# rusty-fast-solvers/rusty-compression

Hardware: AMD Instinct MI355X
Metric: GB/s + compressions/sec, 8192x8192 f64 rank-128 rSVD+ID (higher is better)
Workload: dtype f64

## Files before the change

### bindings/rust/src/ffi.rs

```rust
#![allow(non_camel_case_types)]
use std::os::raw::{c_char, c_void};

pub type rc_status = i32;
pub const RC_OK: rc_status = 0;
pub const RC_LINALG_ERROR: rc_status = 1;
pub const RC_COMPRESSION_ERROR: rc_status = 2;
pub const RC_LAYOUT_ERROR: rc_status = 3;
pub const RC_PIVOTED_QR_ERROR: rc_status = 4;
pub const RC_INVALID_ARGUMENT: rc_status = 5;
pub const RC_RUNTIME_ERROR: rc_status = 6;

pub const RC_PERM_COL: i32 = 0;
pub const RC_PERM_ROW: i32 = 1;
pub const RC_PERM_COLINV: i32 = 2;
pub const RC_PERM_ROWINV: i32 = 3;
pub const RC_VPERM_INV: i32 = 0;
pub const RC_VPERM_NOINV: i32 = 1;

pub const RC_OPT_TALL_SKINNY_FAST_PATH: i32 = 1;
pub const RC_OPT_WIDE_LAZY_QRCP: i32 = 2;
pub const RC_OPT_WIDE_COOP_QRCP: i32 = 3;
pub const RC_OPT_POWER_ITERATION_FIXED: i32 = 4;
pub const RC_OPT_FORK_BRANCHES: i32 = 5;
pub const RC_OPT_BLOCKED_QRCP: i32 = 6;
pub const RC_OPT_CONCURRENCY_HINT: i32 = 7;
pub const RC_OPT_COOP_PANEL: i32 = 8;
pub const RC_OPT_KERNEL_SLOTS: i32 = 9;
pub const RC_OPT_FUSED_CONSUMERS: i32 = 10;

#[repr(C)]
#[derive(Clone, Copy)]
pub struct rc_matrix {
    pub data: *mut c_void,
    pub rows: i64,
    pub cols: i64,
    pub row_stride: i64,
    pub col_stride: i64,
}

#[repr(C)]
#[derive(Clone, Copy)]
pub struct rc_rsvd_id_out {
    pub range_q: rc_matrix,
    pub u: rc_matrix,
    pub s: *mut c_void,
    pub vt: rc_matrix,
    pub qr_q: rc_matrix,
    pub qr_r: rc_matrix,
    pub qr_ind: *mut i64,
    pub id_c: rc_matrix,
    pub id_z: rc_matrix,
}

#[repr(C)]
#[derive(Clone, Copy)]
pub struct rc_complex32 {
    pub re: f32,
    pub im: f32,
}
#[repr(C)]
#[derive(Clone, Copy)]
pub struct rc_complex64 {
    pub re: f64,
    pub im: f64,
}

#[repr(C)]
pub struct rc_context {
    _private: [u8; 0],
}
#[repr(C)]
pub struct rc_comm {
    _private: [u8; 0],
}
pub type rc_host_all_gather_fn = Option<unsafe extern "C" fn(user: *mut c_void, send: *const c_void, recv: *mut c_void, bytes_per_rank: usize) -> i32>;
pub type rc_host_all_reduce_sum_fn = Option<unsafe extern "C" fn(user: *mut c_void, buf: *mut c_void, count: usize, elem_size: i32) -> i32>;
pub type rc_operator_product_fn = Option<unsafe extern "C" fn(user: *mut c_void, ctx: *mut rc_context, x: rc_matrix, y: rc_matrix) -> i32>;
#[repr(C)]
#[derive(Clone, Copy)]
pub struct rc_operator {
    pub rows: i64,
// ... 220 lines not shown
```

### include/rusty_compression_amd.h

```cpp
#ifndef RUSTY_COMPRESSION_AMD_H
#define RUSTY_COMPRESSION_AMD_H

#include <stddef.h>
#include <stdint.h>

#ifdef __cplusplus
extern "C" {
#endif

#define RC_ABI_VERSION 1

typedef int32_t rc_status;
enum {
    RC_OK = 0,
    RC_LINALG_ERROR = 1,
    RC_COMPRESSION_ERROR = 2,
    RC_LAYOUT_ERROR = 3,
    RC_PIVOTED_QR_ERROR = 4,
    RC_INVALID_ARGUMENT = 5,
    RC_RUNTIME_ERROR = 6
};

typedef struct rc_matrix {
    void *data;
    int64_t rows;
    int64_t cols;
    int64_t row_stride;
    int64_t col_stride;
} rc_matrix;

typedef struct rc_context rc_context;

enum { RC_COMPRESS_ADAPTIVE = 0, RC_COMPRESS_RANK = 1 };
enum { RC_PERM_COL = 0, RC_PERM_ROW = 1, RC_PERM_COLINV = 2, RC_PERM_ROWINV = 3 };
enum { RC_VPERM_INV = 0, RC_VPERM_NOINV = 1 };

int32_t rc_abi_version(void);
rc_status rc_create(rc_context **ctx, int32_t device, void *hip_stream);
rc_status rc_destroy(rc_context *ctx);
rc_status rc_set_stream(rc_context *ctx, void *hip_stream);
rc_status rc_stream_create(int32_t device, void **hip_stream);
rc_status rc_stream_destroy(int32_t device, void *hip_stream);
rc_status rc_synchronize(rc_context *ctx);
rc_status rc_synchronize_all(rc_context *const *ctxs, int32_t n);
rc_status rc_reserve_workspace(rc_context *ctx, size_t bytes);
const char *rc_last_error_message(const rc_context *ctx);

rc_status rc_device_malloc(rc_context *ctx, size_t bytes, void **ptr);
rc_status rc_device_free(rc_context *ctx, void *ptr);
rc_status rc_memcpy_h2d(rc_context *ctx, void *dst_dev, const void *src_host, size_t bytes);
rc_status rc_memcpy_d2h(rc_context *ctx, void *dst_host, const void *src_dev, size_t bytes);

rc_status rc_graph_begin_capture(rc_context *ctx);
rc_status rc_graph_end_capture(rc_context *ctx, void **graph_exec);
rc_status rc_graph_launch(rc_context *ctx, void *graph_exec);
rc_status rc_graph_destroy(rc_context *ctx, void *graph_exec);

enum { RC_OPT_TALL_SKINNY_FAST_PATH = 1, RC_OPT_WIDE_LAZY_QRCP = 2, RC_OPT_WIDE_COOP_QRCP = 3, RC_OPT_POWER_ITERATION_FIXED = 4, RC_OPT_FORK_BRANCHES = 5,
       RC_OPT_BLOCKED_QRCP = 6, RC_OPT_CONCURRENCY_HINT = 7, RC_OPT_COOP_PANEL = 8, RC_OPT_KERNEL_SLOTS = 9, RC_OPT_FUSED_CONSUMERS = 10 };
rc_status rc_set_option(rc_context *ctx, int32_t option, int64_t value);
rc_status rc_get_health(rc_context *ctx, int32_t *word);

rc_status rc_profile_enable(rc_context *ctx, int32_t on);
rc_status rc_profile_reset(rc_context *ctx);
rc_status rc_profile_count(rc_context *ctx, int32_t *n);
rc_status rc_profile_get(rc_context *ctx, int32_t i, char *name, int32_t name_cap, double *total_ms, int64_t *calls);

const char *rc_last_gemm_kernel_name(const rc_context *ctx);

rc_status rc_random_gaussian_f64(rc_context *ctx, rc_matrix out, uint64_t seed, uint64_t offset);
rc_status rc_random_gaussian_f32(rc_context *ctx, rc_matrix out, uint64_t seed, uint64_t offset);
rc_status rc_random_bits_u32(rc_context *ctx, uint32_t *out, int64_t n, uint64_t seed, uint64_t word_offset);

rc_status rc_matmat_f64(rc_context *ctx, rc_matrix a, rc_matrix x, rc_matrix y);
rc_status rc_matmat_f32(rc_context *ctx, rc_matrix a, rc_matrix x, rc_matrix y);
rc_status rc_conj_matmat_f64(rc_context *ctx, rc_matrix a, rc_matrix x, rc_matrix y);
rc_status rc_conj_matmat_f32(rc_context *ctx, rc_matrix a, rc_matrix x, rc_matrix y);
rc_status rc_gemm_f64(rc_context *ctx, int32_t trans_a, int32_t trans_b, double alpha, rc_matrix a, rc_matrix b, double beta, rc_matrix c);
rc_status rc_gemm_f32(rc_context *ctx, int32_t trans_a, int32_t trans_b, float alpha, rc_matrix a, rc_matrix b, float beta, rc_matrix c);
rc_status rc_rel_diff_fro_f64(rc_context *ctx, rc_matrix first, rc_matrix second, double *out);
rc_status rc_rel_diff_fro_f32(rc_context *ctx, rc_matrix first, rc_matrix second, float *out);

rc_status rc_invert_permutation(rc_context *ctx, const int64_t *perm, int64_t n, int64_t *inverse);
rc_status rc_apply_permutation_matrix_f64(rc_context *ctx, int32_t mode, rc_matrix in, const int64_t *perm, int64_t perm_len, rc_matrix out);
rc_status rc_apply_permutation_matrix_f32(rc_context *ctx, int32_t mode, rc_matrix in, const int64_t *perm, int64_t perm_len, rc_matrix out);
rc_status rc_apply_permutation_vector_f64(rc_context *ctx, int32_t mode, rc_matrix in, const int64_t *perm, int64_t perm_len, rc_matrix out);
rc_status rc_apply_permutation_vector_f32(rc_context *ctx, int32_t mode, rc_matrix in, const int64_t *perm, int64_t perm_len, rc_matrix out);

rc_status rc_pivoted_qr_f64(rc_context *ctx, rc_matrix a, rc_matrix q, rc_matrix r, int64_t *ind);
rc_status rc_pivoted_qr_f32(rc_context *ctx, rc_matrix a, rc_matrix q, rc_matrix r, int64_t *ind);
rc_status rc_pivoted_lq_f64(rc_context *ctx, rc_matrix a, rc_matrix l, rc_matrix q, int64_t *ind);
rc_status rc_pivoted_lq_f32(rc_context *ctx, rc_matrix a, rc_matrix l, rc_matrix q, int64_t *ind);

rc_status rc_geqp3_f64(rc_context *ctx, rc_matrix a, int64_t kmax, int64_t *jpvt, double *tau);
rc_status rc_geqp3_f32(rc_context *ctx, rc_matrix a, int64_t kmax, int64_t *jpvt, float *tau);
rc_status rc_orgqr_f64(rc_context *ctx, rc_matrix a, const double *tau, int64_t k, rc_matrix q);
rc_status rc_orgqr_f32(rc_context *ctx, rc_matrix a, const float *tau, int64_t k, rc_matrix q);
rc_status rc_trsm_upper_f64(rc_context *ctx, rc_matrix t, rc_matrix b);
rc_status rc_trsm_upper_f32(rc_context *ctx, rc_matrix t, rc_matrix b);

rc_status rc_compute_svd_f64(rc_context *ctx, rc_matrix a, rc_matrix u, double *s, rc_matrix vt);
rc_status rc_compute_svd_f32(rc_context *ctx, rc_matrix a, rc_matrix u, float *s, rc_matrix vt);

rc_status rc_rank_by_tolerance_f64(rc_context *ctx, rc_matrix tri, double tol, int64_t *rank);
rc_status rc_rank_by_tolerance_f32(rc_context *ctx, rc_matrix tri, double tol, int64_t *rank);
rc_status rc_qr_to_mat_f64(rc_context *ctx, rc_matrix q, rc_matrix r, const int64_t *ind, rc_matrix out);
rc_status rc_qr_to_mat_f32(rc_context *ctx, rc_matrix q, rc_matrix r, const int64_t *ind, rc_matrix out);
rc_status rc_lq_to_mat_f64(rc_context *ctx, rc_matrix l, rc_matrix q, const int64_t *ind, rc_matrix out);
rc_status rc_lq_to_mat_f32(rc_context *ctx, rc_matrix l, rc_matrix q, const int64_t *ind, rc_matrix out);
rc_status rc_qr_column_id_f64(rc_context *ctx, rc_matrix q, rc_matrix r, const int64_t *ind, rc_matrix c, rc_matrix z);
rc_status rc_qr_column_id_f32(rc_context *ctx, rc_matrix q, rc_matrix r, const int64_t *ind, rc_matrix c, rc_matrix z);
rc_status rc_lq_row_id_f64(rc_context *ctx, rc_matrix l, rc_matrix q, const int64_t *ind, rc_matrix x, rc_matrix r_rows);
// ... 192 lines not shown
```

### rusty_compression_amd/_lib.py

```python
from __future__ import annotations

import ctypes
import os
import re
import threading
from typing import Dict, Optional, Tuple

_HERE = os.path.dirname(os.path.abspath(__file__))
LIB_PATH = os.path.join(_HERE, "librusty_compression_amd.so")
HEADER_PATH = os.path.join(os.path.dirname(_HERE), "include", "rusty_compression_amd.h")

RC_OPT_TALL_SKINNY_FAST_PATH = 1
RC_OPT_WIDE_LAZY_QRCP = 2
RC_OPT_WIDE_COOP_QRCP = 3
RC_OPT_POWER_ITERATION_FIXED = 4
RC_OPT_FORK_BRANCHES = 5
RC_OPT_BLOCKED_QRCP = 6
RC_OPT_CONCURRENCY_HINT = 7
RC_OPT_COOP_PANEL = 8
RC_OPT_KERNEL_SLOTS = 9
RC_OPT_FUSED_CONSUMERS = 10
RC_OK, RC_LINALG_ERROR, RC_COMPRESSION_ERROR, RC_LAYOUT_ERROR, RC_PIVOTED_QR_ERROR, RC_INVALID_ARGUMENT, RC_RUNTIME_ERROR = range(7)


class RustyCompressionError(Exception):
    """Base of the error enum of the reference (src/types.rs:11-21)."""


class LinalgError(RustyCompressionError):
    pass


class CompressionError(RustyCompressionError):
    """`Could not compress to desired tolerance` (src/types.rs:15-16)."""


class LayoutError(RustyCompressionError):
    pass


class PivotedQRError(RustyCompressionError):
    pass


class HipRuntimeError(RustyCompressionError):
    pass


_STATUS_EXC = {
    RC_LINALG_ERROR: LinalgError,
    RC_COMPRESSION_ERROR: CompressionError,
    RC_LAYOUT_ERROR: LayoutError,
    RC_PIVOTED_QR_ERROR: PivotedQRError,
    RC_INVALID_ARGUMENT: AssertionError,
    RC_RUNTIME_ERROR: HipRuntimeError,
}


class rc_matrix(ctypes.Structure):
    _fields_ = [
        ("data", ctypes.c_void_p),
        ("rows", ctypes.c_int64),
        ("cols", ctypes.c_int64),
        ("row_stride", ctypes.c_int64),
        ("col_stride", ctypes.c_int64),
    ]


class rc_rsvd_id_out(ctypes.Structure):
    _fields_ = [
        ("range_q", rc_matrix),
        ("u", rc_matrix),
        ("s", ctypes.c_void_p),
        ("vt", rc_matrix),
# ... 162 lines not shown
```

### rusty_compression_amd/csrc/kernels_qr.hip

```cpp
#include "rc_common.hpp"
#include "rc_device.hpp"

namespace rc {

static __host__ __device__ inline int64_t cdiv(int64_t a, int64_t b) { return (a + b - 1) / b; }

template <typename T> struct Num;
template <> struct Num<double> {
    static __host__ __device__ inline double tol3z() { return 1.0536712127723509e-08; }
};
template <> struct Num<float> {
    static __host__ __device__ inline float tol3z() { return 2.44140625e-04f; }
};

template <typename T>
__device__ inline T wsum(T v) {
#pragma unroll
    for (int off = 32; off > 0; off >>= 1) v += __shfl_xor(v, off, 64);
    return v;
}

template <typename T, int TPC>
__device__ inline T group_sum(T v, T *sh ) {
    v = wsum(v);
    if (TPC == 256) {
        __syncthreads();
        if ((threadIdx.x & 63) == 0) sh[threadIdx.x >> 6] = v;
        __syncthreads();
        v = sh[0] + sh[1] + sh[2] + sh[3];
    }
    return v;
}

template <typename T>
__global__ __launch_bounds__(256) void k_qr_init(Mat<T> w, int pivot, int64_t *jpvt, T *vn1, T *vn2) {
    __shared__ T sh[4];
    for (int64_t j = blockIdx.x; j < w.cols; j += gridDim.x) {
        if (pivot) {
            const T *col = w.p + j * w.cs;
            T acc = 0;
            for (int64_t i = threadIdx.x; i < w.rows; i += 256) { T v = col[i]; acc += v * v; }
            acc = group_sum<T, 256>(acc, sh);
            if (threadIdx.x == 0) { T nrm = sqrt(acc); vn1[j] = nrm; vn2[j] = nrm; }
        }
        if (threadIdx.x == 0) jpvt[j] = j;
    }
}

template <typename T>
__global__ __launch_bounds__(1024) void k_qr_pivot_reflect(Mat<T> w, int64_t j, int pivot, int64_t *jpvt, T *vn1, T *vn2, T *tau) {
    __shared__ T shv[16];
    __shared__ long long shi[16];
    __shared__ T shs[16];
    const int tid = threadIdx.x, lane = tid & 63, wv = tid >> 6;
// ... 517 lines not shown
__global__ __launch_bounds__(256) void k_id_z(Mat<T> w, const int64_t *jpvt, int64_t k, Mat<T> z) {
    constexpr int NB = 16;
    __shared__ T tile[NB][NB + 1];
    const int64_t n = w.cols;
    const int64_t p = blockIdx.x * (int64_t)blockDim.x + threadIdx.x;
    const bool inside = p < n;
    const int64_t dc = inside ? jpvt[p] : 0;
    const bool active = inside && p >= k;
    const T *bcol = FROM_R ? w.p + (inside ? p : 0) * w.cs : w.p + dc * w.cs;
    const int64_t brs = FROM_R ? w.rs : 1;
    const int64_t nblk = (k + NB - 1) / NB;
    const int ti = threadIdx.x / NB, tj = threadIdx.x % NB;
    if (inside && p < k)
        for (int64_t i = 0; i < k; ++i) z.at(i, dc) = (i == p) ? (T)1 : (T)0;
    for (int64_t bi = nblk - 1; bi >= 0; --bi) {
        const int64_t r0 = bi * NB;
        T acc[NB];
#pragma unroll
        for (int ii = 0; ii < NB; ++ii) acc[ii] = (active && r0 + ii < k) ? bcol[(r0 + ii) * brs] : (T)0;
        for (int64_t bj = nblk - 1; bj >= bi; --bj) {
            const int64_t c0 = bj * NB;
            __syncthreads();
            {
                const int64_t i = r0 + ti, l = c0 + tj;
                tile[ti][tj] = (i < k && l < k && i <= l) ? (FROM_R ? w.at(i, l) : w.p[jpvt[l] * w.cs + i]) : (T)0;
            }
            __syncthreads();
            if (bj > bi) {
                T x[NB];
#pragma unroll
                for (int jj = 0; jj < NB; ++jj) x[jj] = (active && c0 + jj < k) ? z.at(c0 + jj, dc) : (T)0;
#pragma unroll
                for (int jj = 0; jj < NB; ++jj)
#pragma unroll
                    for (int ii = 0; ii < NB; ++ii) acc[ii] -= tile[ii][jj] * x[jj];
            } else {
#pragma unroll
                for (int ii = NB - 1; ii >= 0; --ii) {
                    if (r0 + ii < k) {
                        acc[ii] /= tile[ii][ii];
#pragma unroll
                        for (int i2 = 0; i2 < ii; ++i2) acc[i2] -= tile[i2][ii] * acc[ii];
                    }
                }
            }
        }
        if (active) {
#pragma unroll
            for (int ii = 0; ii < NB; ++ii)
                if (r0 + ii < k) z.at(r0 + ii, dc) = acc[ii];
        }
    }
}
template <typename T>
void column_id_from_qrcp(rc_context *c, Mat<T> a, Mat<T> w, int64_t k, const int64_t *jpvt, Mat<T> cm, Mat<T> z) {
    RC_REQUIRE(w.rs == 1 && a.rows == w.rows && a.cols == w.cols && cm.rows == a.rows && cm.cols == k && z.rows == k && z.cols == a.cols && k <= std::min(a.rows, a.cols),
               RC_INVALID_ARGUMENT, "column_id_from_qrcp: shape mismatch");
    if (a.cols == 0 || k == 0) return;
    ProfScope ps(c, "op:column_id_from_qrcp %lldx%lld k=%lld", (long long)a.rows, (long long)a.cols, (long long)k);
    hipLaunchKernelGGL((k_id_z<T, false>), dim3((unsigned)cdiv(a.cols, 256)), dim3(256), 0, c->stream, w, jpvt, k, z);
    gather_cols(c, a, jpvt, cm);
}
template <typename T>
void id_z_from_r(rc_context *c, Mat<T> r, int64_t k, const int64_t *ind, Mat<T> z) {
    RC_REQUIRE(r.rows == k && z.rows == k && z.cols == r.cols && k <= r.cols, RC_INVALID_ARGUMENT, "id_z_from_r: shape mismatch");
    if (r.cols == 0 || k == 0) return;
    ProfScope ps(c, "op:id_z_from_r k=%lld n=%lld", (long long)k, (long long)r.cols);
    hipLaunchKernelGGL((k_id_z<T, true>), dim3((unsigned)cdiv(r.cols, 256)), dim3(256), 0, c->stream, r, ind, k, z);
}

#define RC_INST(T)                                                                                         \
    template void column_id_from_qrcp<T>(rc_context *, Mat<T>, Mat<T>, int64_t, const int64_t *, Mat<T>, Mat<T>); \
    template void id_z_from_r<T>(rc_context *, Mat<T>, int64_t, const int64_t *, Mat<T>);                 \
    template void geqp3_inplace<T>(rc_context *, Mat<T>, int64_t, bool, int64_t *, T *, T *);             \
    template void extract_r<T>(rc_context *, Mat<T>, const int64_t *, Mat<T>);                             \
    template void form_q<T>(rc_context *, Mat<T>, const int64_t *, const T *, int64_t, Mat<T>);           \
    template void trsm_upper<T>(rc_context *, Mat<T>, Mat<T>);
RC_INST(double)
RC_INST(float)
#undef RC_INST

}

namespace rc {

template <typename T>
__global__ __launch_bounds__(256) void k_wq_init(Mat<T> qacc, Mat<T> rphys) {
    const int64_t tq = qacc.rows * qacc.cols, tr = rphys.rows * rphys.cols;
    for (int64_t e = blockIdx.x * (int64_t)blockDim.x + threadIdx.x; e < tq + tr; e += (int64_t)gridDim.x * blockDim.x) {
        if (e < tq) { int64_t i = e % qacc.rows, c2 = e / qacc.rows; qacc.p[c2 * qacc.cs + i] = (i == c2) ? (T)1 : (T)0; }
        else rphys.p[e - tq] = 0;
    }
}

template <typename T>
__global__ __launch_bounds__(1024) void k_wq_pivot(Mat<T> b, Mat<T> qacc, Mat<T> rphys, int64_t j, int64_t *jpvt, T *vn1, T *vn2, T *tau) {
    extern __shared__ __attribute__((aligned(16))) char smem_raw[];
    const int m = (int)b.rows;
    const int ldq = m | 1;
    long long *shi = reinterpret_cast<long long *>(smem_raw);
    T *shv = reinterpret_cast<T *>(shi + 16);
    T *Q = shv + 16;
    T *bvec = Q + (size_t)m * ldq;
    T *xvec = bvec + m;
    T *vvec = xvec + m;
    T *wvec = vvec + m;
    const int tid = threadIdx.x, lane = tid & 63, wv = tid >> 6;
    const int l8 = tid & 7, g8 = tid >> 3;
    const int64_t n = b.cols;
    const int jj = (int)j;
    for (int e = tid; e < (m - jj) * m; e += 1024) {
        const int i = jj + e / m, r = e % m;
        Q[i * ldq + r] = qacc.p[(int64_t)i * qacc.cs + r];
    }
    {
        T best = (T)-1;
        long long bi = 0x7fffffffffffffffLL;
        for (int64_t p = j + tid; p < n; p += 1024) {
            T v = fabs(vn1[p]);
            if (v > best) { best = v; bi = p; }
        }
// ... 225 lines not shown
```

### rusty_compression_amd/csrc/kernels_tsqr.hip

```cpp
#include "rc_common.hpp"
#include "rc_device.hpp"

namespace rc {

static __host__ __device__ inline int64_t cdiv(int64_t a, int64_t b) { return (a + b - 1) / b; }

template <typename T> struct TNum;
template <> struct TNum<double> {
    static __device__ inline double tol3z() { return 1.0536712127723509e-08; }
    static __device__ inline double tiny() { return 1e-300; }
};
template <> struct TNum<float> {
    static __device__ inline float tol3z() { return 2.44140625e-04f; }
    static __device__ inline float tiny() { return 1e-30f; }
};

template <typename T>
__device__ inline T wave_sum64(T v) {
#pragma unroll
    for (int off = 32; off > 0; off >>= 1) v += __shfl_xor(v, off, 64);
    return v;
}
template <typename T>
__device__ inline T row_sum16(T v) {
// ... 386 lines not shown

template <typename T>
void qrcp_small(rc_context *c, Mat<T> rin, int64_t kmax, bool pivot, int64_t *jpvt, Mat<T> rout, Mat<T> q2) {
    const int64_t n = rin.rows;
    RC_REQUIRE(rin.rows == rin.cols, RC_INVALID_ARGUMENT, "qrcp_small: square input required");
    const size_t lds = ((size_t)n * (n | 1) + 3 * (size_t)n) * sizeof(T) + (size_t)n * sizeof(int) + 64;
    RC_REQUIRE(lds <= 160 * 1024 - 1024 && n <= 208, RC_INVALID_ARGUMENT, "qrcp_small: n = %lld does not fit LDS", (long long)n);
    ProfScope ps(c, "op:qrcp_small n=%lld k=%lld", (long long)n, (long long)kmax);
#define RC_QS(NE, NT_)                                                                                                 \
    do {                                                                                                               \
        auto kern = k_qrcp_small<T, NE, NT_>;                                                                          \
        static bool attr_set[64] = {};                                                                                 \
        if (!attr_set[c->device & 63]) {                                                                               \
            RC_HIP(hipFuncSetAttribute(reinterpret_cast<const void *>(kern), hipFuncAttributeMaxDynamicSharedMemorySize, 160 * 1024 - 1024)); \
            attr_set[c->device & 63] = true;                                                                           \
        }                                                                                                              \
        hipLaunchKernelGGL(kern, dim3(1), dim3(NT_), lds, c->stream, rin, (int)kmax, pivot ? 1 : 0, jpvt, rout, q2);   \
    } while (0)
    static const int wide = [] { const char *e = getenv("RC_QRCP_SMALL_1024"); return e ? atoi(e) : 1; }();
    if (n <= 64) RC_QS(8, 512);
    else if (n <= 144 && wide) RC_QS(18, 1024);
    else if (n <= 144) RC_QS(18, 512);
    else RC_QS(26, 512);
#undef RC_QS
}

template <typename T>
__global__ __launch_bounds__(1024) void k_householder_signs(Mat<T> q, T *d) {
    extern __shared__ __attribute__((aligned(16))) char smem_raw[];
    const int k = (int)q.cols;
    const int ld = k | 1;
    T *W = reinterpret_cast<T *>(smem_raw);
    const int tid = threadIdx.x;
    for (int e = tid; e < k * k; e += 1024) {
        int i = e % k, cc = e / k;
        W[i * ld + cc] = q.at(i, cc);
    }
    __syncthreads();
    const int ti = tid >> 5, tc = tid & 31;
    for (int j = 0; j < k; ++j) {
        const T s = W[j * ld + j];
        const T dj = (s > (T)0) ? (T)-1 : (T)1;
        const T u = (T)1 + fabs(s);
        if (tid == 0) d[j] = dj;
        const T inv = -dj / u;
        for (int i = j + 1 + ti; i < k; i += 32) {
            const T li = W[i * ld + j] * inv;
            for (int cc = j + 1 + tc; cc < k; cc += 32) W[i * ld + cc] -= li * W[j * ld + cc];
        }
        __syncthreads();
    }
}
template <typename T>
__global__ __launch_bounds__(256) void k_scale_cols_rows(Mat<T> q, Mat<T> r, const T *d) {
    const int64_t tq = q.rows * q.cols, tr = r.rows * r.cols;
    for (int64_t e = blockIdx.x * (int64_t)blockDim.x + threadIdx.x; e < tq + tr; e += (int64_t)gridDim.x * blockDim.x) {
        if (e < tq) {
            int64_t j = e / q.rows, i = e - j * q.rows;
            if (d[j] < (T)0) q.at(i, j) = -q.at(i, j);
        } else {
            int64_t f = e - tq;
            int64_t i = f / r.cols, p = f - i * r.cols;
            if (d[i] < (T)0) r.at(i, p) = -r.at(i, p);
        }
    }
}

template <typename T>
static void householder_signs(rc_context *c, Mat<T> top, T *d) {
    const int64_t k = top.cols;
    const size_t lds = (size_t)k * (k | 1) * sizeof(T);
    RC_REQUIRE(top.rows >= k && lds <= 160 * 1024 - 1024, RC_INVALID_ARGUMENT, "sign fix: k = %lld does not fit LDS", (long long)k);
    auto kern = k_householder_signs<T>;
    static bool attr_set[64] = {};
    if (!attr_set[c->device & 63]) {
        RC_HIP(hipFuncSetAttribute(reinterpret_cast<const void *>(kern), hipFuncAttributeMaxDynamicSharedMemorySize, 160 * 1024 - 1024));
        attr_set[c->device & 63] = true;
    }
    hipLaunchKernelGGL(kern, dim3(1), dim3(1024), lds, c->stream, top, d);
}
template <typename T>
static void scale_cols_rows(rc_context *c, Mat<T> q, Mat<T> r, const T *d) {
    const int64_t total = q.rows * q.cols + r.rows * r.cols;
    hipLaunchKernelGGL(k_scale_cols_rows<T>, dim3((unsigned)std::min<int64_t>(cdiv(total, 256), 4096)), dim3(256), 0, c->stream, q, r, d);
}

template <typename T>
void householder_sign_fix(rc_context *c, Mat<T> q, Mat<T> r) {
    const int64_t k = q.cols;
    if (k == 0) return;
    RC_REQUIRE(q.rows >= k, RC_INVALID_ARGUMENT, "sign fix: q must be tall");
    ProfScope ps(c, "op:householder_sign_fix k=%lld", (long long)k);
    ArenaMark mark(c);
    T *d = c->alloc<T>((size_t)k);
    householder_signs<T>(c, q, d);
    scale_cols_rows<T>(c, q, r, d);
}

template <typename T>
void qrcp_tall_fast(rc_context *c, Mat<T> y, int64_t k, bool pivot, Mat<T> q, Mat<T> r, int64_t *ind, int *flag) {
    const int64_t m = y.rows, n = y.cols;
    ProfScope ps(c, "op:qrcp_tall_fast %lldx%lld k=%lld pivot=%d", (long long)m, (long long)n, (long long)k, pivot ? 1 : 0);
    ArenaMark mark(c);
    static const int fold = [] { const char *e = getenv("RC_TSQR_FOLD"); return e ? atoi(e) : 1; }();
    Mat<T> q1 = rowmajor(c->alloc<T>((size_t)m * even_ld(n)), m, n, even_ld(n));
    Mat<T> r1 = colmajor(c->alloc<T>((size_t)n * even_ld(n)), n, n, even_ld(n));
    Mat<T> r2i = rowmajor(c->alloc<T>((size_t)n * even_ld(n)), n, n, even_ld(n));
    if (fold) tsqr_cholqr2_factored<T>(c, y, q1, r2i, r1, flag);
    else tsqr_cholqr2<T>(c, y, q1, r1, flag);
    Mat<T> q2 = colmajor(c->alloc<T>((size_t)even_ld(n) * k), n, k, even_ld(n));
    Mat<T> rr = r.empty() ? rowmajor(c->alloc<T>((size_t)k * even_ld(n)), k, n, even_ld(n)) : r;
    qrcp_small<T>(c, r1, k, pivot, ind, rr, q2);
    Mat<T> qq = q.empty() ? rowmajor(c->alloc<T>((size_t)m * even_ld(k)), m, k, even_ld(k)) : q;
    if (!fold) {
        gemm<T>(c, 1, q1, q2, 0, qq);
        householder_sign_fix<T>(c, qq, rr);
        return;
    }
    Mat<T> w = colmajor(c->alloc<T>((size_t)even_ld(n) * k), n, k, even_ld(n));
    Mat<T> top = colmajor(c->alloc<T>((size_t)even_ld(k) * k), k, k, even_ld(k));
    T *d = c->alloc<T>((size_t)k);
    gemm<T>(c, 1, r2i, q2, 0, w);
    gemm<T>(c, 1, q1.sub(0, k, 0, n), w, 0, top);
    householder_signs<T>(c, top, d);
    scale_cols_rows<T>(c, w, rr, d);
    gemm<T>(c, 1, q1, w, 0, qq);
}

#define RC_INST(T)                                                                                               \
    template bool tsqr_supported<T>(int64_t, int64_t);                                                           \
    template void tsqr_cholqr2<T>(rc_context *, Mat<T>, Mat<T>, Mat<T>, int *);                                  \
    template void tsqr_cholqr2_factored<T>(rc_context *, Mat<T>, Mat<T>, Mat<T>, Mat<T>, int *);                 \
// ... 9 lines not shown
```

### rusty_compression_amd/csrc/rc_api.hip

```cpp
#include "rc_common.hpp"

#include <unistd.h>

#include <atomic>
#include <chrono>

#include <algorithm>
#include <cmath>

using namespace rc;

static constexpr size_t kAlign = 256;

void rc_context::retire_arena() {
    if (arena) {
        if (live_graphs > 0) retired.push_back(arena);
        else (void)hipFree(arena);
    }
    arena = nullptr;
    arena_size = 0;
}

void rc_context::swap_arena() {
    std::swap(arena, aux_arena.base);
// ... 1283 lines not shown
    if (e != hipSuccess) { ctx->last_error = hipGetErrorString(e); return RC_RUNTIME_ERROR; }
    ctx->capturing = true;
    return RC_OK;
}
rc_status rc_graph_end_capture(rc_context *ctx, void **graph_exec) {
    if (!ctx || !graph_exec) return RC_INVALID_ARGUMENT;
    DeviceGuard dg(ctx->device);
    *graph_exec = nullptr;
    hipGraph_t graph = nullptr;
    hipError_t e = hipStreamEndCapture(ctx->stream, &graph);
    ctx->capturing = false;
    if (e != hipSuccess || !graph) { ctx->last_error = std::string("hipStreamEndCapture: ") + hipGetErrorString(e); return RC_RUNTIME_ERROR; }
    hipGraphExec_t exec = nullptr;
    e = hipGraphInstantiate(&exec, graph, nullptr, nullptr, 0);
    (void)hipGraphDestroy(graph);
    if (e != hipSuccess) { ctx->last_error = std::string("hipGraphInstantiate: ") + hipGetErrorString(e); return RC_RUNTIME_ERROR; }
    *graph_exec = exec;
    ctx->live_graphs += 1;
    return RC_OK;
}
rc_status rc_graph_launch(rc_context *ctx, void *graph_exec) {
    if (!ctx || !graph_exec) return RC_INVALID_ARGUMENT;
    DeviceGuard dg(ctx->device);
    hipError_t e = hipGraphLaunch(static_cast<hipGraphExec_t>(graph_exec), ctx->stream);
    if (e != hipSuccess) { ctx->last_error = hipGetErrorString(e); return RC_RUNTIME_ERROR; }
    return RC_OK;
}
rc_status rc_graph_destroy(rc_context *ctx, void *graph_exec) {
    if (!ctx) return RC_INVALID_ARGUMENT;
    if (!graph_exec) return RC_OK;
    DeviceGuard dg(ctx->device);
    (void)hipStreamSynchronize(ctx->stream);
    (void)hipGraphExecDestroy(static_cast<hipGraphExec_t>(graph_exec));
    if (ctx->live_graphs > 0 && --ctx->live_graphs == 0) {
        for (void *p : ctx->retired) (void)hipFree(p);
        ctx->retired.clear();
    }
    return RC_OK;
}

rc_status rc_set_option(rc_context *ctx, int32_t option, int64_t value) {
    if (!ctx) return RC_INVALID_ARGUMENT;
    switch (option) {
        case RC_OPT_TALL_SKINNY_FAST_PATH: ctx->opt_tsqr = value != 0; return RC_OK;
        case RC_OPT_WIDE_LAZY_QRCP: ctx->opt_wide_lazy = value != 0; return RC_OK;
        case RC_OPT_WIDE_COOP_QRCP: ctx->opt_wide_coop = value != 0; return RC_OK;
        case RC_OPT_POWER_ITERATION_FIXED: ctx->opt_power_fixed = value != 0; return RC_OK;
        case RC_OPT_FORK_BRANCHES: ctx->opt_fork = value != 0; return RC_OK;
        case RC_OPT_BLOCKED_QRCP: ctx->opt_blocked = value != 0; return RC_OK;
        case RC_OPT_COOP_PANEL: ctx->opt_coop_panel = value != 0; return RC_OK;
        case RC_OPT_CONCURRENCY_HINT: ctx->opt_lanes = (int)std::max<int64_t>(1, std::min<int64_t>(value, 1024)); return RC_OK;
        case RC_OPT_KERNEL_SLOTS: ctx->opt_slots = (int)std::max<int64_t>(1, std::min<int64_t>(value, 1024)); return RC_OK;
        case RC_OPT_FUSED_CONSUMERS: ctx->opt_fused_consumers = value != 0; return RC_OK;
        default: ctx->last_error = "unknown option"; return RC_INVALID_ARGUMENT;
    }
}
rc_status rc_get_health(rc_context *ctx, int32_t *word) {
    if (!ctx || !word) return RC_INVALID_ARGUMENT;
    DeviceGuard dg(ctx->device);
    *word = 0;
    if (!ctx->health) return RC_OK;
    int h = 0;
    if (debug_memset_path() & 2) {
        hipError_t e = hipStreamSynchronize(ctx->stream);
        if (e == hipSuccess) e = hipMemcpy(&h, ctx->health, sizeof(int), hipMemcpyDeviceToHost);
        if (e == hipSuccess) e = hipMemset(ctx->health, 0, sizeof(int));
        if (e != hipSuccess) { ctx->last_error = hipGetErrorString(e); return RC_RUNTIME_ERROR; }
        *word = h;
        return RC_OK;
    }
    try {
        read_back(ctx, ctx->health, &h, 1);
        hipLaunchKernelGGL(k_set_word, dim3(1), dim3(64), 0, ctx->stream, ctx->health, 0);
        RC_HIP(hipStreamSynchronize(ctx->stream));
    } catch (const Error &e) { ctx->last_error = e.msg; return e.code; }
    *word = h;
    return RC_OK;
}

rc_status rc_profile_enable(rc_context *ctx, int32_t on) {
    if (!ctx) return RC_INVALID_ARGUMENT;
    ctx->prof_on = on != 0;
    return RC_OK;
}
rc_status rc_profile_reset(rc_context *ctx) {
    if (!ctx) return RC_INVALID_ARGUMENT;
    DeviceGuard dg(ctx->device);
    ctx->prof_resolve();
    ctx->prof_acc.clear();
    return RC_OK;
}
rc_status rc_profile_count(rc_context *ctx, int32_t *n) {
    if (!ctx || !n) return RC_INVALID_ARGUMENT;
    DeviceGuard dg(ctx->device);
    ctx->prof_resolve();
    *n = (int32_t)ctx->prof_acc.size();
    return RC_OK;
}
rc_status rc_profile_get(rc_context *ctx, int32_t i, char *name, int32_t name_cap, double *total_ms, int64_t *calls) {
    if (!ctx || i < 0 || i >= (int32_t)ctx->prof_acc.size()) return RC_INVALID_ARGUMENT;
    auto it = ctx->prof_acc.begin();
    std::advance(it, i);
    if (name && name_cap > 0) {
        std::strncpy(name, it->first.c_str(), (size_t)name_cap - 1);
        name[name_cap - 1] = 0;
    }
// ... 284 lines not shown
```

### rusty_compression_amd/csrc/rc_common.hpp

```cpp
#pragma once

#include <hip/hip_runtime.h>

#include <cstdarg>
#include <cstdint>
#include <cstdio>
#include <cstring>
#include <map>
#include <string>
#include <vector>

#include "../../include/rusty_compression_amd.h"

namespace rc {

template <typename T>
struct Mat {
    T *p = nullptr;
    int64_t rows = 0, cols = 0, rs = 0, cs = 0;

    __host__ __device__ Mat() {}
    __host__ __device__ Mat(T *p_, int64_t r, int64_t c, int64_t rs_, int64_t cs_) : p(p_), rows(r), cols(c), rs(rs_), cs(cs_) {}
    __host__ __device__ inline T &at(int64_t i, int64_t j) const { return p[i * rs + j * cs]; }
    __host__ __device__ Mat<T> sub(int64_t r0, int64_t nr, int64_t c0, int64_t nc) const {
// ... 25 lines not shown
    vsnprintf(buf, sizeof(buf), fmt, ap);
    va_end(ap);
    throw Error{code, std::string(buf)};
}

#define RC_HIP(expr)                                                                                   \
    do {                                                                                               \
        hipError_t _e = (expr);                                                                        \
        if (_e != hipSuccess) ::rc::fail(RC_RUNTIME_ERROR, "%s failed: %s (%s:%d)", #expr,             \
                                         hipGetErrorString(_e), __FILE__, __LINE__);                   \
    } while (0)

#define RC_REQUIRE(cond, code, ...)                  \
    do {                                             \
        if (!(cond)) ::rc::fail(code, __VA_ARGS__);  \
    } while (0)

}

struct rc_context {
    int device = 0;
    hipStream_t stream = nullptr;
    std::string last_error;
    std::string last_gemm_kernel;

    int call_depth = 0;
    char *arena = nullptr;
    size_t arena_size = 0;
    size_t arena_off = 0;
    size_t arena_high = 0;
    std::vector<void *> overflow;
    int live_graphs = 0;
    std::vector<void *> retired;
    void retire_arena();
    hipStream_t aux_stream = nullptr;
    hipEvent_t fork_ev = nullptr, join_ev = nullptr;
    struct ArenaState { char *base = nullptr; size_t size = 0, off = 0, high = 0; std::vector<void *> overflow; } aux_arena;
    void swap_arena();
    int opt_fork = 0;
    hipEvent_t sync_ev = nullptr;
    void *pinned = nullptr;
    size_t pinned_size = 0;
    int pinned_cursor = 0;

    int opt_tsqr = 1;
    int opt_power_fixed = 0;
    int opt_wide_coop = 1;
    int opt_wide_lazy = 1;
    int opt_blocked = 1;
    int opt_coop_panel = 1;
    int opt_lanes = 1;
    int opt_slots = 4;
    int opt_fused_consumers = 1;
    int lanes_in_flight() const { return opt_lanes < opt_slots ? opt_lanes : opt_slots; }
    int *health = nullptr;
    int *health_word();
    unsigned *epoch = nullptr;
    unsigned *epoch_word();

    bool capturing = false;
    bool prof_on = false;
    struct ProfPending { std::string name; hipEvent_t beg, end; };
    struct ProfAcc { double ms = 0; int64_t calls = 0; };
    std::vector<ProfPending> prof_pending;
    std::vector<hipEvent_t> prof_free;
    std::map<std::string, ProfAcc> prof_acc;
    hipEvent_t prof_event();
    void prof_resolve();

    void reset_arena();
    void *alloc_bytes(size_t bytes);
    template <typename T>
    T *alloc(size_t n) { return static_cast<T *>(alloc_bytes(n * sizeof(T))); }
    void reserve(size_t bytes);
    void release_all();
};

namespace rc {

struct ProfScope {
    rc_context *c;
    hipEvent_t beg = nullptr;
    std::string name;
    ProfScope(rc_context *ctx, const char *fmt, ...) : c(ctx) {
        if (!c->prof_on || c->capturing) return;
        char buf[160];
        va_list ap;
        va_start(ap, fmt);
        vsnprintf(buf, sizeof(buf), fmt, ap);
        va_end(ap);
        name = buf;
        beg = c->prof_event();
        (void)hipEventRecord(beg, c->stream);
    }
    ~ProfScope() {
        if (!beg) return;
        hipEvent_t end = c->prof_event();
        (void)hipEventRecord(end, c->stream);
        c->prof_pending.push_back({name, beg, end});
    }
};

struct ArenaMark {
    rc_context *c;
    size_t off;
    explicit ArenaMark(rc_context *ctx) : c(ctx), off(ctx->arena_off) {}
// ... 95 lines not shown
```

Before: 662.4.

## Add LDS-tiled ID back-substitution and blocked Householder sign-fix kernels

Adds a new option, on by default, that selects two restructured small kernels. The interpolative-decomposition Z solve becomes a blocked back-substitution: 16x16 tiles of the triangular factor are staged in LDS with the next tile prefetched, and each thread keeps its solved vector in LDS. The single-block Householder sign-fix kernel becomes a panel-blocked version that does the panel factorisation with wavefront lane reads and then a register-blocked trailing update. Both aim to cut global and LDS traffic in these serial small-k steps, at the cost of large dynamic LDS use and smaller blocks (64 threads) for the ID kernel.

```diff
diff --git a/bindings/rust/src/ffi.rs b/bindings/rust/src/ffi.rs
--- a/bindings/rust/src/ffi.rs
+++ b/bindings/rust/src/ffi.rs
@@ -27,6 +27,7 @@
 pub const RC_OPT_COOP_PANEL: i32 = 8;
 pub const RC_OPT_KERNEL_SLOTS: i32 = 9;
 pub const RC_OPT_FUSED_CONSUMERS: i32 = 10;
+pub const RC_OPT_SMALL_SCHEDULES: i32 = 11;
 
 #[repr(C)]
 #[derive(Clone, Copy)]
diff --git a/include/rusty_compression_amd.h b/include/rusty_compression_amd.h
--- a/include/rusty_compression_amd.h
+++ b/include/rusty_compression_amd.h
@@ -57,7 +57,8 @@
 rc_status rc_graph_destroy(rc_context *ctx, void *graph_exec);
 
 enum { RC_OPT_TALL_SKINNY_FAST_PATH = 1, RC_OPT_WIDE_LAZY_QRCP = 2, RC_OPT_WIDE_COOP_QRCP = 3, RC_OPT_POWER_ITERATION_FIXED = 4, RC_OPT_FORK_BRANCHES = 5,
-       RC_OPT_BLOCKED_QRCP = 6, RC_OPT_CONCURRENCY_HINT = 7, RC_OPT_COOP_PANEL = 8, RC_OPT_KERNEL_SLOTS = 9, RC_OPT_FUSED_CONSUMERS = 10 };
+       RC_OPT_BLOCKED_QRCP = 6, RC_OPT_CONCURRENCY_HINT = 7, RC_OPT_COOP_PANEL = 8, RC_OPT_KERNEL_SLOTS = 9, RC_OPT_FUSED_CONSUMERS = 10,
+       RC_OPT_SMALL_SCHEDULES = 11 };
 rc_status rc_set_option(rc_context *ctx, int32_t option, int64_t value);
 rc_status rc_get_health(rc_context *ctx, int32_t *word);
 
diff --git a/rusty_compression_amd/_lib.py b/rusty_compression_amd/_lib.py
--- a/rusty_compression_amd/_lib.py
+++ b/rusty_compression_amd/_lib.py
@@ -20,6 +20,7 @@
 RC_OPT_COOP_PANEL = 8
 RC_OPT_KERNEL_SLOTS = 9
 RC_OPT_FUSED_CONSUMERS = 10
+RC_OPT_SMALL_SCHEDULES = 11
 RC_OK, RC_LINALG_ERROR, RC_COMPRESSION_ERROR, RC_LAYOUT_ERROR, RC_PIVOTED_QR_ERROR, RC_INVALID_ARGUMENT, RC_RUNTIME_ERROR = range(7)
 
 
diff --git a/rusty_compression_amd/csrc/kernels_qr.hip b/rusty_compression_amd/csrc/kernels_qr.hip
--- a/rusty_compression_amd/csrc/kernels_qr.hip
+++ b/rusty_compression_amd/csrc/kernels_qr.hip
@@ -1,5 +1,6 @@
 #include "rc_common.hpp"
 #include "rc_device.hpp"
+#include <type_traits>
 
 namespace rc {
 
@@ -623,13 +624,104 @@
         }
     }
 }
+template <typename T, bool FROM_R>
+__global__ __launch_bounds__(64) void k_id_z_lds(Mat<T> w, const int64_t *jpvt, int64_t k, Mat<T> z) {
+    constexpr int NB = 16, NTH = 64, PER = NB * NB / NTH;
+    extern __shared__ __attribute__((aligned(16))) char smem_raw[];
+    T *xs = reinterpret_cast<T *>(smem_raw);
+    T(*tile)[NB + 1] = reinterpret_cast<T(*)[NB + 1]>(xs + (size_t)k * NTH);
+    const int tid = threadIdx.x;
+    const int64_t n = w.cols;
+    const int64_t p = blockIdx.x * (int64_t)NTH + tid;
+    const bool inside = p < n;
+    const int64_t dc = inside ? jpvt[p] : 0;
+    const bool active = inside && p >= k;
+    const T *bcol = FROM_R ? w.p + (inside ? p : 0) * w.cs : w.p + dc * w.cs;
+    const int64_t brs = FROM_R ? w.rs : 1;
+    const int64_t nblk = (k + NB - 1) / NB;
+    if (inside && p < k)
+        for (int64_t i = 0; i < k; ++i) z.at(i, dc) = (i == p) ? (T)1 : (T)0;
+    if (blockIdx.x * (int64_t)NTH + NTH <= k) return;
+    T nxt[PER];
+    auto fetch = [&](int64_t bi, int64_t bj) {
+#pragma unroll
+        for (int e = 0; e < PER; ++e) {
+            const int idx = tid + NTH * e;
+            const int64_t i = bi * NB + idx / NB, l = bj * NB + idx % NB;
+            nxt[e] = (i < k && l < k && i <= l) ? (FROM_R ? w.at(i, l) : w.p[jpvt[l] * w.cs + i]) : (T)0;
+        }
+    };
+    fetch(nblk - 1, nblk - 1);
+    for (int64_t bi = nblk - 1; bi >= 0; --bi) {
+        const int64_t r0 = bi * NB;
+        T acc[NB];
+#pragma unroll
+        for (int ii = 0; ii < NB; ++ii) acc[ii] = (active && r0 + ii < k) ? bcol[(r0 + ii) * brs] : (T)0;
+        for (int64_t bj = nblk - 1; bj >= bi; --bj) {
+            const int64_t c0 = bj * NB;
+            __syncthreads();
+#pragma unroll
+            for (int e = 0; e < PER; ++e) {
+                const int idx = tid + NTH * e;
+                tile[idx / NB][idx % NB] = nxt[e];
+            }
+            __syncthreads();
+            if (bj > bi) fetch(bi, bj - 1);
+            else if (bi > 0) fetch(bi - 1, nblk - 1);
+            if (bj > bi) {
+                T x[NB];
+#pragma unroll
+                for (int jj = 0; jj < NB; ++jj) x[jj] = (active && c0 + jj < k) ? xs[(c0 + jj) * NTH + tid] : (T)0;
+#pragma unroll
+                for (int jj = 0; jj < NB; ++jj)
+#pragma unroll
+                    for (int ii = 0; ii < NB; ++ii) acc[ii] = fma(-tile[ii][jj], x[jj], acc[ii]);
+            } else {
+#pragma unroll
+                for (int ii = NB - 1; ii >= 0; --ii) {
+                    if (r0 + ii < k) {
+                        acc[ii] /= tile[ii][ii];
+#pragma unroll
+                        for (int i2 = 0; i2 < ii; ++i2) acc[i2] = fma(-tile[i2][ii], acc[ii], acc[i2]);
+                    }
+                }
+            }
+        }
+        if (active) {
+#pragma unroll
+            for (int ii = 0; ii < NB; ++ii)
+                if (r0 + ii < k) {
+                    z.at(r0 + ii, dc) = acc[ii];
+                    if (bi > 0) xs[(r0 + ii) * NTH + tid] = acc[ii];
+                }
+        }
+    }
+}
+template <typename T>
+static size_t id_z_lds_bytes(int64_t k) { return ((size_t)k * 64 + 16 * 17) * sizeof(T); }
+template <typename T, bool FROM_R>
+static void id_z_launch(rc_context *c, Mat<T> w, const int64_t *jpvt, int64_t k, Mat<T> z) {
+    if constexpr (std::is_same<T, double>::value) {
+        if (c->opt_small_schedules && id_z_lds_bytes<T>(k) <= 160 * 1024 - 1024) {
+            auto kern = k_id_z_lds<T, FROM_R>;
+            static bool attr_set[64] = {};
+            if (!attr_set[c->device & 63]) {
+                RC_HIP(hipFuncSetAttribute(reinterpret_cast<const void *>(kern), hipFuncAttributeMaxDynamicSharedMemorySize, 160 * 1024 - 1024));
+                attr_set[c->device & 63] = true;
+            }
+            hipLaunchKernelGGL(kern, dim3((unsigned)cdiv(w.cols, 64)), dim3(64), id_z_lds_bytes<T>(k), c->stream, w, jpvt, k, z);
+            return;
+        }
+    }
+    hipLaunchKernelGGL((k_id_z<T, FROM_R>), dim3((unsigned)cdiv(w.cols, 256)), dim3(256), 0, c->stream, w, jpvt, k, z);
+}
 template <typename T>
 void column_id_from_qrcp(rc_context *c, Mat<T> a, Mat<T> w, int64_t k, const int64_t *jpvt, Mat<T> cm, Mat<T> z) {
     RC_REQUIRE(w.rs == 1 && a.rows == w.rows && a.cols == w.cols && cm.rows == a.rows && cm.cols == k && z.rows == k && z.cols == a.cols && k <= std::min(a.rows, a.cols),
                RC_INVALID_ARGUMENT, "column_id_from_qrcp: shape mismatch");
     if (a.cols == 0 || k == 0) return;
     ProfScope ps(c, "op:column_id_from_qrcp %lldx%lld k=%lld", (long long)a.rows, (long long)a.cols, (long long)k);
-    hipLaunchKernelGGL((k_id_z<T, false>), dim3((unsigned)cdiv(a.cols, 256)), dim3(256), 0, c->stream, w, jpvt, k, z);
+    id_z_launch<T, false>(c, w, jpvt, k, z);
     gather_cols(c, a, jpvt, cm);
 }
 template <typename T>
@@ -637,7 +729,7 @@
     RC_REQUIRE(r.rows == k && z.rows == k && z.cols == r.cols && k <= r.cols, RC_INVALID_ARGUMENT, "id_z_from_r: shape mismatch");
     if (r.cols == 0 || k == 0) return;
     ProfScope ps(c, "op:id_z_from_r k=%lld n=%lld", (long long)k, (long long)r.cols);
-    hipLaunchKernelGGL((k_id_z<T, true>), dim3((unsigned)cdiv(r.cols, 256)), dim3(256), 0, c->stream, r, ind, k, z);
+    id_z_launch<T, true>(c, r, ind, k, z);
 }
 
 #define RC_INST(T)                                                                                         \
diff --git a/rusty_compression_amd/csrc/kernels_tsqr.hip b/rusty_compression_amd/csrc/kernels_tsqr.hip
--- a/rusty_compression_amd/csrc/kernels_tsqr.hip
+++ b/rusty_compression_amd/csrc/kernels_tsqr.hip
@@ -462,6 +462,93 @@
     }
 }
 template <typename T>
+__global__ __launch_bounds__(1024) void k_householder_signs_panel(Mat<T> q, T *d) {
+    constexpr int NB = 8, AB = 4;
+    extern __shared__ __attribute__((aligned(16))) char smem_raw[];
+    const int k = (int)q.cols;
+    const int ld = k | 1;
+    T *W = reinterpret_cast<T *>(smem_raw);
+    const int tid = threadIdx.x;
+    for (int e = tid; e < k * k; e += 1024) {
+        int i = e % k, cc = e / k;
+        W[i * ld + cc] = q.at(i, cc);
+    }
+    __syncthreads();
+    const int lane = tid & 63, wv = tid >> 6;
+    const int ti = tid >> 5, tc = tid & 31;
+    for (int j0 = 0; j0 < k; j0 += NB) {
+        const int nb = min(NB, k - j0);
+        const int b0 = j0 + nb;
+        const int ns = (k - b0 + 63) >> 6;
+        const int nrow = max(ns, 1);
+        if (wv < nrow + ns) {
+            const bool isrow = wv < nrow;
+            const int e = b0 + 64 * (isrow ? wv : wv - nrow) + lane;
+            const bool live = e < k;
+            T D[NB], P[NB];
+#pragma unroll
+            for (int r = 0; r < NB; ++r) {
+                D[r] = (r < nb && lane < nb) ? W[(j0 + r) * ld + j0 + lane] : (T)0;
+                P[r] = (r < nb && live) ? (isrow ? W[(j0 + r) * ld + e] : W[e * ld + j0 + r]) : (T)0;
+            }
+#pragma unroll
+            for (int jj = 0; jj < NB; ++jj) {
+                if (jj < nb) {
+                    const T s = read_lane(D[jj], jj);
+                    const T dj = (s > (T)0) ? (T)-1 : (T)1;
+                    const T u = (T)1 + fabs(s);
+                    if (tid == 0) d[j0 + jj] = dj;
+                    const T inv = -dj / u;
+                    const T li = P[jj] * inv;
+#pragma unroll
+                    for (int r = jj + 1; r < NB; ++r) {
+                        const T lr = read_lane(D[r], jj) * inv;
+                        const T wjr = read_lane(D[jj], r);
+                        P[r] = isrow ? fma(-lr, P[jj], P[r]) : fma(-li, wjr, P[r]);
+                        D[r] = (lane > jj) ? fma(-lr, D[jj], D[r]) : D[r];
+                    }
+                    if (!isrow) P[jj] = li;
+                }
+            }
+            if (live) {
+#pragma unroll
+                for (int r = 0; r < NB; ++r)
+                    if (r < nb) {
+                        if (isrow) W[(j0 + r) * ld + e] = P[r];
+                        else W[e * ld + j0 + r] = P[r];
+                    }
+            }
+        }
+        if (b0 >= k) break;
+        __syncthreads();
+        for (int a0 = b0 + ti; a0 < k; a0 += 32 * AB) {
+            T L[AB][NB];
+#pragma unroll
+            for (int qa = 0; qa < AB; ++qa) {
+                const int i = a0 + 32 * qa;
+#pragma unroll
+                for (int jj = 0; jj < NB; ++jj) L[qa][jj] = (i < k) ? W[i * ld + j0 + jj] : (T)0;
+            }
+            for (int cc = b0 + tc; cc < k; cc += 32) {
+                T rw[NB];
+#pragma unroll
+                for (int jj = 0; jj < NB; ++jj) rw[jj] = W[(j0 + jj) * ld + cc];
+#pragma unroll
+                for (int qa = 0; qa < AB; ++qa) {
+                    const int i = a0 + 32 * qa;
+                    if (i < k) {
+                        T w = W[i * ld + cc];
+#pragma unroll
+                        for (int jj = 0; jj < NB; ++jj) w = fma(-L[qa][jj], rw[jj], w);
+                        W[i * ld + cc] = w;
+                    }
+                }
+            }
+        }
+        __syncthreads();
+    }
+}
+template <typename T>
 __global__ __launch_bounds__(256) void k_scale_cols_rows(Mat<T> q, Mat<T> r, const T *d) {
     const int64_t tq = q.rows * q.cols, tr = r.rows * r.cols;
     for (int64_t e = blockIdx.x * (int64_t)blockDim.x + threadIdx.x; e < tq + tr; e += (int64_t)gridDim.x * blockDim.x) {
@@ -482,12 +569,14 @@
     const size_t lds = (size_t)k * (k | 1) * sizeof(T);
     RC_REQUIRE(top.rows >= k && lds <= 160 * 1024 - 1024, RC_INVALID_ARGUMENT, "sign fix: k = %lld does not fit LDS", (long long)k);
     auto kern = k_householder_signs<T>;
+    auto kern_panel = k_householder_signs_panel<T>;
     static bool attr_set[64] = {};
     if (!attr_set[c->device & 63]) {
         RC_HIP(hipFuncSetAttribute(reinterpret_cast<const void *>(kern), hipFuncAttributeMaxDynamicSharedMemorySize, 160 * 1024 - 1024));
+        RC_HIP(hipFuncSetAttribute(reinterpret_cast<const void *>(kern_panel), hipFuncAttributeMaxDynamicSharedMemorySize, 160 * 1024 - 1024));
         attr_set[c->device & 63] = true;
     }
-    hipLaunchKernelGGL(kern, dim3(1), dim3(1024), lds, c->stream, top, d);
+    hipLaunchKernelGGL(c->opt_small_schedules ? kern_panel : kern, dim3(1), dim3(1024), lds, c->stream, top, d);
 }
 template <typename T>
 static void scale_cols_rows(rc_context *c, Mat<T> q, Mat<T> r, const T *d) {
diff --git a/rusty_compression_amd/csrc/rc_api.hip b/rusty_compression_amd/csrc/rc_api.hip
--- a/rusty_compression_amd/csrc/rc_api.hip
+++ b/rusty_compression_amd/csrc/rc_api.hip
@@ -1359,6 +1359,7 @@
         case RC_OPT_CONCURRENCY_HINT: ctx->opt_lanes = (int)std::max<int64_t>(1, std::min<int64_t>(value, 1024)); return RC_OK;
         case RC_OPT_KERNEL_SLOTS: ctx->opt_slots = (int)std::max<int64_t>(1, std::min<int64_t>(value, 1024)); return RC_OK;
         case RC_OPT_FUSED_CONSUMERS: ctx->opt_fused_consumers = value != 0; return RC_OK;
+        case RC_OPT_SMALL_SCHEDULES: ctx->opt_small_schedules = value != 0; return RC_OK;
         default: ctx->last_error = "unknown option"; return RC_INVALID_ARGUMENT;
     }
 }
diff --git a/rusty_compression_amd/csrc/rc_common.hpp b/rusty_compression_amd/csrc/rc_common.hpp
--- a/rusty_compression_amd/csrc/rc_common.hpp
+++ b/rusty_compression_amd/csrc/rc_common.hpp
@@ -101,6 +101,7 @@
     int opt_lanes = 1;
     int opt_slots = 4;
     int opt_fused_consumers = 1;
+    int opt_small_schedules = 1;
     int lanes_in_flight() const { return opt_lanes < opt_slots ? opt_lanes : opt_slots; }
     int *health = nullptr;
     int *health_word();
```

Result: no change. 661.0 (-0.2%).
